# TaihuLight/Lol

Measured on AMD Instinct MI355X. Metric: cyclotomic poly-muls/sec (CRT·pointwise·CRT⁻¹), batched; bit-exact vs CT, higher is better.
Workload: dtype u64

## Files before the change

lol_amd/csrc/capi.cpp:

```cpp
#include <hip/hip_runtime_api.h>

#include <atomic>
#include <cstdlib>
#include <cstring>
#include <map>
#include <memory>
#include <mutex>
#include <string>
#include <vector>

#include "kernels.h"
#include "she_host.h"

using namespace lolhip;

namespace lolhip {
namespace {
const char* const kSwitchNames[SW_COUNT] = {"GENERIC_SCALAR", "NO_FUSED2", "NO_POW2_PART", "POLYMUL_UNFUSED",
                                            "KEYSWITCH_UNFUSED", "NO_T1", "NO_PIPE", "FORCE_PIPE", "NO_OWN_DIAG", "NO_MERGE", "NO_LAZY", "NO_KRON", "NO_TRUNC", "ELT_GLOBAL", "LPRF_VALU", "RLWE_RING_UNFUSED", "GAUSS_DENSE", "ZQ_DENSE_VALU", "ZQ_DENSE_MFMA", "CPLX_DENSE", "CPLX_DENSE_VALU", "ZQ_SCAN"};
std::atomic<int> g_switch[SW_COUNT];
std::once_flag g_switch_once;
void switches_init() {
  std::call_once(g_switch_once, [] {
    for (int i = 0; i < SW_COUNT; ++i) {
// ... 77 lines not shown
int zq_dense_route(const Plan& P, const StageProgram& sp) {
  if (!(P.routes & LOLHIP_ROUTE_DENSE_ZQ) || P.zq_mats.empty() || sw(SW_GENERIC_SCALAR)) return 0;
  if (use_mixed(P, sp) || sp.stages.size() > (size_t)ZQ_MAX_STAGES) return 0;
  int dmax = 0;
  for (const Stage& st : sp.stages) if (zq_dense_stage(st) && st.d > dmax) dmax = st.d;
  if (!dmax) return 0;
  return (P.zq_W && (dmax >= ZQ_MFMA_MIN_D || sw(SW_ZQ_DENSE_MFMA)) && !sw(SW_ZQ_DENSE_VALU)) ? 2 : 1;
}
const ZqDenseMat* zq_mat_of(const Plan& P, const Stage& st) {
  if (zq_dense_stage(st)) for (const ZqDenseMat& zm : P.zq_mats) if (zm.mat_off == st.mat_off) return &zm;
  return nullptr;
}

void zq_fill(const Plan& P, const StageProgram& sp, size_t at, ZqDenseLaunch& z) {
  z.W = P.zq_W; z.fold = P.zq_fold;
  z.mt = P.d_zq_mt; z.mtpc = P.zq_mt_per_comp;
  z.planes = P.d_zq_planes; z.plpc = P.zq_pl_per_comp;
  for (size_t i = 0; i < sp.stages.size(); ++i) {
    const Stage& st = sp.stages[i];
    const ZqDenseMat* zm = zq_mat_of(P, st);
    if (zm && st.d > z.dmax) z.dmax = st.d;
    z.kind[at + i] = !zm ? ZQ_ELT : st.rts >= 64 ? ZQ_COLS : ZQ_ROWS;
    z.mt_off[at + i] = zm ? zm->mt_off : -1; z.dp[at + i] = zm ? zm->dp : 0; z.pl_off[at + i] = zm ? zm->pl_off : -1;
  }
}

int zq_scan_route(const Plan& P, const StageProgram& sp) {
  if (!(P.routes & LOLHIP_ROUTE_SCAN_ZQ) || sw(SW_GENERIC_SCALAR) || P.n > 8192) return 0;
  const bool forced = sw(SW_ZQ_SCAN);
  if ((!forced && use_mixed(P, sp)) || sp.stages.size() > (size_t)ZQ_MAX_STAGES) return 0;
  bool hit = false;
  for (const Stage& st : sp.stages) {
    if (zq_scan_stage(st)) hit = hit || st.p > 13 || forced;
    else if (st.kind != ST_DIAG && st.kind != ST_SCALE) return 0;
  }
  return hit ? 1 : 0;
}

bool q_below(const Plan& P, int bits) {
  for (u64 q : P.qs) if (q >> bits) return false;
  return true;
}

bool use_fused2(const Plan& P) {
  return !sw(SW_NO_FUSED2) && P.fused2 && use_mixed(P, P.prog_crt_fused) && use_mixed(P, P.prog_crtinv_fused);
}

int run_pow2(const Plan& P, int mode, hipStream_t s, int64_t* y, const int64_t* a, const int64_t* b, int64_t B) {
  Pow2Launch l;
  l.stream = s; l.y = y; l.a = a; l.b = b; l.B = B; l.T = P.T; l.L = P.pow2.L;
  l.mod = P.d_mod;
  if (P.pow2.arith32) {
    l.arith = P.pow2.arith32; l.tw_fwd = P.pow2.d_tw_fwd32; l.tw_inv = P.pow2.d_tw_inv32; l.scale = P.pow2.d_scale32;
  } else {
    l.arith = 1;
    for (u64 q : P.qs) if (q >= (1ull << 61) || !(q & 1)) l.arith = 0;
    l.tw_fwd = P.pow2.d_tw_fwd; l.tw_inv = P.pow2.d_tw_inv; l.scale = P.pow2.d_scale;
    l.trunc = (l.arith == 1 && mode == 2 && !sw(SW_NO_TRUNC)) ? 1 : 0;
  }
  return hip_status(launch_pow2(l, mode));
}

}

namespace lolhip {

int need_device(const Plan& P) {
  if (!P.device) return LOLHIP_ERR_NO_DEVICE;
  int dev = -1;
  if (hipGetDevice(&dev) != hipSuccess) return LOLHIP_ERR_HIP;
  if (dev != P.device_id) return LOLHIP_ERR_DEVICE;
  return LOLHIP_OK;
}

int need_device(const lolhip_plan* p) { return p ? need_device(p->P) : LOLHIP_ERR_INVALID; }

int run_prog(const Plan& P, const StageProgram& sp, hipStream_t s, int64_t* y, int64_t B, const int64_t* src) {
  const int scan = zq_scan_route(P, sp);
  if (!scan && use_mixed(P, sp)) return hip_status(launch_mixed(mixed_launch(P, s, y, src ? src : y, B, sp)));
  GenericLaunch a;
  a.stream = s; a.y = y; a.B = B; a.T = P.T; a.n = P.n;
  a.stages = sp.d_stages; a.nstages = sp.nstages;
  a.consts = P.d_consts; a.cpc = P.consts_per_comp; a.mod = P.d_mod;
  StreamBuf ring(s);
  a.scratch = nullptr; a.scratch_bytes = 0;
  if (P.needs_scratch && B > 0) {
    const i64 groups = B * P.T < 512 ? B * P.T : 512;
    a.scratch_bytes = (size_t)groups * 2 * (size_t)P.n * sizeof(u64);
    if (!ring.alloc(a.scratch_bytes)) return LOLHIP_ERR_HIP;
    a.scratch = (u64*)ring.p;
  }
  a.q32 = true;
  for (u64 q : P.qs) if (q >= ((u64)1 << 32)) a.q32 = false;
  if (scan) {
    a.scan.route = scan;
    a.scan.src = (src && src != y) ? src : nullptr;
    a.scan.host_stages = sp.stages.data();
    for (size_t i = 0; i < sp.stages.size(); ++i)
      a.scan.kind[i] = !zq_scan_stage(sp.stages[i]) ? ZS_ELT : sp.stages[i].rts >= 64 ? ZS_COLS : ZS_LANES;
    return hip_status(launch_generic(a));
  }
  a.zq.route = zq_dense_route(P, sp);
  if (a.zq.route) {
    zq_fill(P, sp, 0, a.zq);
    a.zq.src = (src && src != y) ? src : nullptr;
    return hip_status(launch_generic(a));
// ... 919 lines not shown
```

lol_amd/csrc/plan.cpp:

```cpp
#include "plan.h"

#include <hip/hip_runtime_api.h>

#include <cmath>
#include <complex>
#include <cstring>

#include "kernels.h"
#include "lolhip.h"

namespace lolhip {

namespace {

template <typename E>
struct PoolBuilderT {
  int T;
  std::vector<std::vector<E>> pool;
  explicit PoolBuilderT(int T_) : T(T_), pool((size_t)T_) {}
  int size() const { return (int)pool[0].size(); }
  int add(const std::vector<std::vector<E>>& tab) {
    int off = size();
    for (int t = 0; t < T; ++t) pool[(size_t)t].insert(pool[(size_t)t].end(), tab[(size_t)t].begin(), tab[(size_t)t].end());
    return off;
// ... 743 lines not shown
    const Stage& st = P.prog_gauss.stages[si];
    if (st.wp_off) P.prog_gauss.nstages |= (st.rts >= 64 ? GAUSS_COLS : GAUSS_ROWS) << (8 + 2 * (int)si);
  }
  if ((rc = P.d_gcrt.upload(P.gcrt))) return rc;
  if ((rc = P.d_ginvcrt.upload(P.ginvcrt))) return rc;
  if ((rc = P.d_lift.upload(P.lift_consts))) return rc;

  if (P.is_pow2 || P.pow2_part) {
    const int L = P.pow2.L;
    const i64 n = (i64)1 << L;
    std::vector<u64> fwd((size_t)(T * n * 2), 0), inv((size_t)(T * n * 2), 0), sc((size_t)(T * 12), 0);
    for (int t = 0; t < T; ++t) {
      const u64 q = P.qs[(size_t)t];
      const u64 S = (u64)P.mhatinv[(size_t)t];
      {
        const u64 w1 = mulmod((u64)P.ruinv[0][(size_t)((n >> 1) * T + t)], S, q);
        const u64 R = (u64)((((unsigned __int128)1) << 64) % q);
        const u64 vals[4] = {S, w1, mulmod(S, R, q), mulmod(w1, R, q)};
        for (int k = 0; k < 4; ++k) {
          ShoupW ss = make_shoup(vals[k], q);
          sc[(size_t)(t * 8 + 2 * k)] = ss.w; sc[(size_t)(t * 8 + 2 * k + 1)] = ss.wp;
        }
        if (L >= 2) {
          const u64 S4 = mulmod(vals[2], 4 % q, q);
          const u64 tv[2] = {S4, mulmod(vals[3], 4 % q, q)};
          for (int k = 0; k < 2; ++k) {
            ShoupW ss = make_shoup(tv[k], q);
            sc[(size_t)(T * 8 + t * 4 + 2 * k)] = ss.w; sc[(size_t)(T * 8 + t * 4 + 2 * k + 1)] = ss.wp;
          }
        }
      }
      for (int s = 1; s <= L; ++s) {
        const i64 N = (i64)1 << s, half = N >> 1, step = n / N;
        for (i64 i = 0; i < half; ++i) {
          const i64 ex = step * (2 * i + 1);
          u64 w = (u64)P.ru[0][(size_t)(ex * T + t)];
          u64 wi = (u64)P.ruinv[0][(size_t)(ex * T + t)];
          if (s == 1) wi = mulmod(wi, S, q);
          ShoupW a = make_shoup(w, q), b = make_shoup(wi, q);
          const size_t o = ((size_t)t * n + (size_t)(half + i)) * 2;
          fwd[o] = a.w; fwd[o + 1] = a.wp;
          inv[o] = b.w; inv[o + 1] = b.wp;
        }
      }
    }
    if ((rc = P.pow2.d_tw_fwd.upload(fwd))) return rc;
    if ((rc = P.pow2.d_tw_inv.upload(inv))) return rc;
    if ((rc = P.pow2.d_scale.upload(sc))) return rc;
    P.pow2.arith32 = 4;
    for (u64 q : P.qs) { if (q >= (1ull << 27)) P.pow2.arith32 = 2; }
    for (u64 q : P.qs) { if (q >= (1ull << 30)) P.pow2.arith32 = 3; }
    for (u64 q : P.qs) { if (q >= (1ull << 31) || !(q & 1)) P.pow2.arith32 = 0; }
    if (P.pow2.arith32) {
      std::vector<uint32_t> f32(fwd.size()), i32(inv.size()), s32((size_t)T * 8);
      for (int t = 0; t < T; ++t) {
        const u64 q = P.qs[(size_t)t];
        for (i64 i = 0; i < n; ++i) {
          const size_t o = ((size_t)t * n + (size_t)i) * 2;
          f32[o] = (uint32_t)fwd[o]; f32[o + 1] = (uint32_t)((fwd[o] << 32) / q);
          i32[o] = (uint32_t)inv[o]; i32[o + 1] = (uint32_t)((inv[o] << 32) / q);
        }
        for (int k = 0; k < 4; ++k) {
          s32[(size_t)t * 8 + 2 * k] = (uint32_t)sc[(size_t)t * 8 + 2 * k];
          s32[(size_t)t * 8 + 2 * k + 1] = (uint32_t)((sc[(size_t)t * 8 + 2 * k] << 32) / q);
        }
      }
      if ((rc = P.pow2.d_tw_fwd32.upload(f32))) return rc;
      if ((rc = P.pow2.d_tw_inv32.upload(i32))) return rc;
      if ((rc = P.pow2.d_scale32.upload(s32))) return rc;
    }
  }
  P.needs_scratch = 2 * (size_t)P.n * sizeof(u64) > 152 * 1024;
  if (P.mixed_cls == 2 || P.mixed_cls == 4 || P.mixed_cls == 3) {
    const int sh = P.mixed_cls == 3 ? 64 : 32;
    std::vector<u64> mont(P.host_consts.size());
    for (int t = 0; t < T; ++t) {
      const u64 q = P.qs[(size_t)t];
      const u64 r = (u64)((((unsigned __int128)1) << sh) % q);
      for (int i = 0; i < P.consts_per_comp; ++i) {
        const size_t o = (size_t)t * P.consts_per_comp + i;
        mont[o] = mulmod(P.host_consts[o] % q, r, q);
      }
    }
    if ((rc = P.d_consts_mont.upload(mont))) return rc;
    if (P.mixed_cls == 2 || P.mixed_cls == 4) {
      std::vector<uint32_t> c32(mont.begin(), mont.end());
      if ((rc = P.d_consts32.upload(c32))) return rc;
    }
  }
  if (P.mixed_cls == 1) {
    std::vector<uint32_t> c32(P.host_consts.size());
    for (int t = 0; t < T; ++t)
      for (int i = 0; i < P.consts_per_comp; ++i) {
        const size_t o = (size_t)t * P.consts_per_comp + i;
        c32[o] = (uint32_t)(P.host_consts[o] % P.qs[(size_t)t]);
      }
    if ((rc = P.d_consts32.upload(c32))) return rc;
  }
  if (hipGetDevice(&P.device_id) != hipSuccess) return LOLHIP_ERR_HIP;
  P.device = true;
  return LOLHIP_OK;
}

}
```

lol_amd/csrc/pow2_impl.h:

```cpp
#pragma once
#include <hip/hip_runtime.h>

#include <atomic>
#include <mutex>
#include <type_traits>
#include <utility>

#include "kernels.h"
#include "zq_dev.h"

namespace lolhip {


constexpr int R = 4;
constexpr int E = 1 << R;
constexpr int LEVEL_PARTS = 4;

struct Lay {
  int reg[R];
  int thr[12];
  int ntb;
};
constexpr bool lay_eq(const Lay& a, const Lay& b) {
  if (a.ntb != b.ntb) return false;
// ... 489 lines not shown
    if (L < 10) return lay_std(L, L - R);
    int thr[12] = {0, 1, 2, 3, 4, 5, 10, 11, 12, 13, 14, 15};
    return lay_make(L, 6, 7, 8, 9, thr);
  }
  static constexpr Lay final_layout() { return HAS_G ? g() : wave_end(); }
};

template <int AR, bool INV, Lay A, int K0, int K1 = R>
__device__ __forceinline__ void fetch4(LevelTwT<VT<AR>> (&t)[R], const TwCtxT<VT<AR>>& tw, int xt) {
  if constexpr (K0 <= 0 && K1 > 0) tw_fetch<INV, A, 0>(t[0], tw, xt);
  if constexpr (K0 <= 1 && K1 > 1) tw_fetch<INV, A, 1>(t[1], tw, xt);
  if constexpr (K0 <= 2 && K1 > 2) tw_fetch<INV, A, 2>(t[2], tw, xt);
  if constexpr (K0 <= 3 && K1 > 3) tw_fetch<INV, A, 3>(t[3], tw, xt);
}
template <int AR, bool INV, Lay A, int K>
__device__ __forceinline__ void level_jit(VT<AR> (&v)[E], const TwCtxT<VT<AR>>& tw, int xt, const auto& qk) {
  using LevelTw = LevelTwT<VT<AR>>;
  if constexpr (tw_distinct(A, K) == 8 && sizeof(VT<AR>) == 8) {
    [&]<int... PART>(std::integer_sequence<int, PART...>) {
      (([&] { LevelTw t; tw_fetch<INV, A, K, PART>(t, tw, xt); level<AR, INV, A, K, PART>(v, t, tw, qk); }()), ...);
    }(std::make_integer_sequence<int, LEVEL_PARTS>{});
  } else {
    LevelTw t; tw_fetch<INV, A, K>(t, tw, xt); level<AR, INV, A, K>(v, t, tw, qk);
  }
}
template <int AR, Lay A, int K0, int K1 = R>
__device__ __forceinline__ void levels4_jit(VT<AR> (&v)[E], const TwCtxT<VT<AR>>& tw, int xt, const auto& qk) {
  if constexpr (K0 <= 0 && K1 > 0) level_jit<AR, false, A, 0>(v, tw, xt, qk);
  if constexpr (K0 <= 1 && K1 > 1) level_jit<AR, false, A, 1>(v, tw, xt, qk);
  if constexpr (K0 <= 2 && K1 > 2) level_jit<AR, false, A, 2>(v, tw, xt, qk);
  if constexpr (K0 <= 3 && K1 > 3) level_jit<AR, false, A, 3>(v, tw, xt, qk);
}
template <int AR, bool INV, Lay A, int K0, int K1 = R>
__device__ __forceinline__ void levels4(VT<AR> (&v)[E], const LevelTwT<VT<AR>> (&t)[R], const TwCtxT<VT<AR>>& tw, const auto& qk) {
  if constexpr (!INV) {
    if constexpr (K0 <= 0 && K1 > 0) level<AR, false, A, 0>(v, t[0], tw, qk);
    if constexpr (K0 <= 1 && K1 > 1) level<AR, false, A, 1>(v, t[1], tw, qk);
    if constexpr (K0 <= 2 && K1 > 2) level<AR, false, A, 2>(v, t[2], tw, qk);
    if constexpr (K0 <= 3 && K1 > 3) level<AR, false, A, 3>(v, t[3], tw, qk);
  } else {
    if constexpr (K0 <= 3 && K1 > 3) level<AR, true, A, 3>(v, t[3], tw, qk);
    if constexpr (K0 <= 2 && K1 > 2) level<AR, true, A, 2>(v, t[2], tw, qk);
    if constexpr (K0 <= 1 && K1 > 1) level<AR, true, A, 1>(v, t[1], tw, qk);
    if constexpr (K0 <= 0 && K1 > 0) level<AR, true, A, 0>(v, t[0], tw, qk);
  }
}

__device__ __forceinline__ int fresh(int x) {
  asm volatile("" : "+v"(x));
  return x;
}

struct NoTop {};
template <int AR, int L, Lay PREV, bool LEAN = false, bool W16 = false, typename TOP = NoTop, bool TRUNC = false>
__device__ __forceinline__ void fwd_transform(VT<AR> (&v)[E], VT<AR>* lds, const TwCtxT<VT<AR>>& tw, int tau_in, const auto& qk,
                                              TOP* pre = nullptr) {
  constexpr bool PRE = !std::is_same_v<TOP, NoTop>;
  using LevelTw = LevelTwT<VT<AR>>;
  using S = Sched<L, W16>;
  static_assert(!TRUNC || (L >= 11 && !PRE), "the truncated forward transform needs the G layout");
  constexpr int GK1 = TRUNC ? 2 : R;
  constexpr bool L10 = !(TRUNC && L == 11);
  {
    constexpr Lay A = S::w0();
    const int tau = fresh(tau_in);
    if constexpr (S::HAS_G && !lay_eq(PREV, A)) __syncthreads();
    transpose_put<PREV, A, false>(v, lds, tau);
    if constexpr (LEAN) {
      transpose_get<PREV, A, false>(v, lds, tau);
      levels4_jit<AR, A, 0>(v, tw, xthr<A>(tau), qk);
    } else {
      LevelTw t[R];
      fetch4<AR, false, A, 0>(t, tw, xthr<A>(tau));
      transpose_get<PREV, A, false>(v, lds, tau);
      levels4<AR, false, A, 0>(v, t, tw, qk);
    }
  }
  if constexpr (S::HAS_W1) {
    constexpr Lay A = S::w1();
    const int tau = fresh(tau_in);
    if constexpr (LEAN) {
      transpose_put<S::w0(), A, false>(v, lds, tau);
      transpose_get<S::w0(), A, false>(v, lds, tau);
      levels4_jit<AR, A, S::W1_K0>(v, tw, xthr<A>(tau), qk);
      if constexpr (S::NSWAP >= 1) { lane_swap<4, 3>(v); level_jit<AR, false, S::w1a(), 3>(v, tw, xthr<S::w1a()>(tau), qk); }
      if constexpr (S::NSWAP >= 2) {
        lane_swap<5, 2>(v);
        if constexpr (PRE) { pre->wait_l10(); level<AR, false, S::w1b(), 2>(v, pre->l10, tw, qk); }
        else if constexpr (L10) level_jit<AR, false, S::w1b(), 2>(v, tw, xthr<S::w1b()>(tau), qk);
      }
    } else {
      LevelTw t[R];
      transpose_put<S::w0(), A, false>(v, lds, tau);
      fetch4<AR, false, A, S::W1_K0>(t, tw, xthr<A>(tau));
      transpose_get<S::w0(), A, false>(v, lds, tau);
      if constexpr (S::W1_K0 <= 0) level<AR, false, A, 0>(v, t[0], tw, qk);
      if constexpr (S::W1_K0 <= 1) level<AR, false, A, 1>(v, t[1], tw, qk);
      if constexpr (S::W1_K0 <= 2) level<AR, false, A, 2>(v, t[2], tw, qk);
      LevelTw ua, ub;
      if constexpr (S::NSWAP >= 1) tw_fetch<false, S::w1a(), 3>(ua, tw, xthr<S::w1a()>(tau));
      level<AR, false, A, 3>(v, t[3], tw, qk);
      if constexpr (S::NSWAP >= 2 && !PRE && L10) tw_fetch<false, S::w1b(), 2>(ub, tw, xthr<S::w1b()>(tau));
      if constexpr (S::NSWAP >= 1) { lane_swap<4, 3>(v); level<AR, false, S::w1a(), 3>(v, ua, tw, qk); }
      if constexpr (S::NSWAP >= 2) {
        lane_swap<5, 2>(v);
        if constexpr (PRE) { pre->wait_l10(); level<AR, false, S::w1b(), 2>(v, pre->l10, tw, qk); }
        else if constexpr (L10) level<AR, false, S::w1b(), 2>(v, ub, tw, qk);
      }
    }
  }
  if constexpr (S::HAS_G) {
    constexpr Lay A = S::g();
    const int tau = fresh(tau_in);
    transpose_put<S::wave_end(), A, false>(v, lds, tau);
    if constexpr (PRE) {
      transpose_get<S::wave_end(), A, true>(v, lds, tau);
      pre->wait_g();
      levels4<AR, false, A, S::G_K0>(v, pre->g, tw, qk);
    } else if constexpr (LEAN) {
      transpose_get<S::wave_end(), A, true>(v, lds, tau);
      levels4_jit<AR, A, S::G_K0, GK1>(v, tw, xthr<A>(tau), qk);
    } else {
      LevelTw t[R];
      fetch4<AR, false, A, S::G_K0, GK1>(t, tw, xthr<A>(tau));
      transpose_get<S::wave_end(), A, true>(v, lds, tau);
      levels4<AR, false, A, S::G_K0, GK1>(v, t, tw, qk);
    }
  }
}

template <int AR, int L, Lay NEXT, bool W16 = false, bool TRUNC = false>
__device__ __forceinline__ void inv_transform(VT<AR> (&v)[E], VT<AR>* lds, const TwCtxT<VT<AR>>& tw, int tau_in, const auto& qk) {
  using LevelTw = LevelTwT<VT<AR>>;
  using S = Sched<L, W16>;
  static_assert(!TRUNC || L >= 11, "the truncated inverse transform needs the G layout");
  constexpr int GK1 = TRUNC ? 2 : R;
  constexpr bool L10 = !(TRUNC && L == 11);
  if constexpr (S::HAS_G) {
    constexpr Lay A = S::g();
    const int tau = fresh(tau_in);
    LevelTw t[R];
    fetch4<AR, true, A, S::G_K0, GK1>(t, tw, xthr<A>(tau));
    levels4<AR, true, A, S::G_K0, GK1>(v, t, tw, qk);
    transpose_put<A, S::wave_end(), true>(v, lds, tau);
  }
  if constexpr (S::HAS_W1) {
    constexpr Lay A = S::w1();
    const int tau = fresh(tau_in);
    const int xt = xthr<A>(tau);
    LevelTw ua, ub, t[R];
    if constexpr (S::NSWAP >= 2 && L10) tw_fetch<true, S::w1b(), 2>(ub, tw, xthr<S::w1b()>(tau));
    if constexpr (S::NSWAP >= 1) tw_fetch<true, S::w1a(), 3>(ua, tw, xthr<S::w1a()>(tau));
    if constexpr (S::NSWAP == 0) fetch4<AR, true, A, S::W1_K0>(t, tw, xt);
    if constexpr (S::HAS_G) transpose_get<S::g(), S::wave_end(), true>(v, lds, tau);
    if constexpr (S::NSWAP >= 2) { if constexpr (L10) level<AR, true, S::w1b(), 2>(v, ub, tw, qk); lane_swap<5, 2>(v); }
    if constexpr (S::NSWAP >= 1) {
      tw_fetch<true, A, 3>(t[3], tw, xt);
      level<AR, true, S::w1a(), 3>(v, ua, tw, qk);
      lane_swap<4, 3>(v);
      tw_fetch<true, A, 2>(t[2], tw, xt);
      tw_fetch<true, A, 1>(t[1], tw, xt);
      tw_fetch<true, A, 0>(t[0], tw, xt);
    }
    levels4<AR, true, A, S::W1_K0>(v, t, tw, qk);
    transpose_put<A, S::w0(), false>(v, lds, tau);
  }
  {
    constexpr Lay A = S::w0();
    const int tau = fresh(tau_in);
    LevelTw t[R];
    fetch4<AR, true, A, 0>(t, tw, xthr<A>(tau));
    if constexpr (S::HAS_W1) transpose_get<S::w1(), A, false>(v, lds, tau);
    levels4<AR, true, A, 0>(v, t, tw, qk);
    transpose_put<A, NEXT, false>(v, lds, tau);
    transpose_get<A, NEXT, false>(v, lds, tau);
  }
}


__device__ __forceinline__ void dot4_cols(const u64 (&x)[4], const u64 (&y)[4], u64& A, u64& B1, u64& B2, u64& C) {
  u64 k1, k2, k3, sj;
  u32 cnt;
  asm("v_mad_u64_u32 %[C], %[sj], %[x0l], %[y0l], 0\n\t"
      "v_mad_u64_u32 %[A], %[sj], %[x0h], %[y0h], 0\n\t"
      "v_mad_u64_u32 %[B1], %[sj], %[x0l], %[y0h], 0\n\t"
      "v_mad_u64_u32 %[C], %[k1], %[x1l], %[y1l], %[C]\n\t"
      "v_mad_u64_u32 %[B2], %[sj], %[x0h], %[y0l], 0\n\t"
      "v_mad_u64_u32 %[A], %[sj], %[x1h], %[y1h], %[A]\n\t"
      "v_cndmask_b32_e64 %[cnt], 0, 1, %[k1]\n\t"
      "v_mad_u64_u32 %[C], %[k2], %[x2l], %[y2l], %[C]\n\t"
// ... 1 lines not shown
      "v_mad_u64_u32 %[B2], %[sj], %[x1h], %[y1l], %[B2]\n\t"
      "v_addc_co_u32_e64 %[cnt], %[sj], %[cnt], 0, %[k2]\n\t"
      "v_mad_u64_u32 %[C], %[k3], %[x3l], %[y3l], %[C]\n\t"
      "v_mad_u64_u32 %[A], %[sj], %[x2h], %[y2h], %[A]\n\t"
      "v_mad_u64_u32 %[B1], %[sj], %[x2l], %[y2h], %[B1]\n\t"
      "v_addc_co_u32_e64 %[cnt], %[sj], %[cnt], 0, %[k3]\n\t"
      "v_mad_u64_u32 %[B2], %[sj], %[x2h], %[y2l], %[B2]\n\t"
      "v_mad_u64_u32 %[A], %[sj], %[x3h], %[y3h], %[A]\n\t"
      "v_mad_u64_u32 %[B1], %[sj], %[x3l], %[y3h], %[B1]\n\t"
      "v_mad_u64_u32 %[B2], %[sj], %[x3h], %[y3l], %[B2]\n\t"
      "v_mad_u64_u32 %[A], %[sj], %[cnt], 1, %[A]"
      : [A] "=&v"(A), [B1] "=&v"(B1), [B2] "=&v"(B2), [C] "=&v"(C), [cnt] "=&v"(cnt),
        [k1] "=&s"(k1), [k2] "=&s"(k2), [k3] "=&s"(k3), [sj] "=&s"(sj)
      : [x0l] "v"(lo32(x[0])), [x0h] "v"(hi32(x[0])), [x1l] "v"(lo32(x[1])), [x1h] "v"(hi32(x[1])),
        [x2l] "v"(lo32(x[2])), [x2h] "v"(hi32(x[2])), [x3l] "v"(lo32(x[3])), [x3h] "v"(hi32(x[3])),
        [y0l] "v"(lo32(y[0])), [y0h] "v"(hi32(y[0])), [y1l] "v"(lo32(y[1])), [y1h] "v"(hi32(y[1])),
        [y2l] "v"(lo32(y[2])), [y2h] "v"(hi32(y[2])), [y3l] "v"(lo32(y[3])), [y3h] "v"(hi32(y[3])));
}
__device__ __forceinline__ u64 dot4_redc(const u64 (&x)[4], const u64 (&y)[4], const ModCtx& mc) {
  u64 A, B1, B2, C;
  dot4_cols(x, y, A, B1, B2, C);
  const u64 u = (u64)hi32(C) + lo32(B1) + lo32(B2);
  const u64 lo = ((u64)lo32(u) << 32) | lo32(C);
  const u64 hi = A + hi32(B1) + hi32(B2) + hi32(u);
  return hi + __umul64hi(lo * mc.nqinv, mc.q) + (lo != 0);
}
template <Lay G>
__device__ __forceinline__ void pow2_base4(u64 (&v)[E], const u64 (&va)[E], const TwCtxT<u64>& tw, int xt, const ModCtx& mc, const QK& qk) {
  LevelTwT<u64> z;
  tw_fetch<false, G, 1>(z, tw, xt);
#pragma unroll
  for (int g = 0; g < 4; ++g) {
    constexpr int EK[4] = {0, 8, 4, 12};
    u64 zw = z.w[level_tab<G, 1>.slot[g & 1]], zwp = z.wp[level_tab<G, 1>.slot[g & 1]];
    if (g & 2) { zw = qk.q - zw; zwp = ~zwp; }
    u64 a[4], y[4];
#pragma unroll
    for (int k = 0; k < 4; ++k) {
      a[k] = va[g | EK[k]];
      y[k] = trim42(v[g | EK[k]], qk);
    }
#pragma unroll
    for (int k = 3; k >= 0; --k) {
      u64 x[4], w[4];
#pragma unroll
      for (int i = 0; i < 4; ++i) { x[i] = a[i]; w[i] = y[(k - i) & 3]; }
      v[g | EK[k]] = dot4_redc(x, w, mc);
      asm volatile("" : "+v"(v[g | EK[k]]));
      if (k) y[k] = trim2(shoup_acc<false>(y[k], zw, zwp, qk.nq, 0), qk);
    }
  }
}

constexpr int pow2_threads(int L) { return (1 << (L - R)) >= 256 ? (1 << (L - R)) : 256; }

template <int L, int MODE, int AR, bool T1 = false, bool TR = false>
__global__ void __launch_bounds__(pow2_threads(L), AR >= 2 ? 8 : 4)
k_pow2(i64* y, const i64* a_in, const i64* b_in, i64 B, int T,
       const VT<AR>* __restrict__ tw_fwd, const VT<AR>* __restrict__ tw_inv, const VT<AR>* __restrict__ scale,
       const ModCtx* __restrict__ mod, int xcd_map) {
  using S = Sched<L, T1>;
  using V = VT<AR>;
  static_assert(!TR || (MODE == 2 && AR == 1 && L >= 11), "the truncated route is the 61-bit fused poly-mul's");
  constexpr int n = 1 << L;
  constexpr int NT = 1 << (L - R);
  constexpr int PPW = NT >= 256 ? 1 : 256 / NT;
  constexpr int LDSW = n + n / 16 + twl_words(n);
  constexpr u32 TWB = 2 * sizeof(V);
  extern __shared__ __attribute__((aligned(16))) unsigned char smem[];
  V* lds = reinterpret_cast<V*>(smem) + (threadIdx.x / NT) * LDSW;
  V* lds_tw = lds + n + n / 16;
  const int tau = threadIdx.x % NT;
  if constexpr (T1) T = 1;

  const i64 item0 = (i64)blockIdx.x * PPW;
  const int slot = (PPW == 1) ? 0 : (int)(threadIdx.x / NT);
  const i64 item = item0 + slot;
  i64 b, b0; int t;
  if (xcd_map) { i64 g = item / (8 * (i64)T); int r = (int)(item % (8 * T)); b = g * 8 + (r & 7); t = r >> 3; b0 = b; }
  else { b = item / T; t = (int)(item % T); b0 = item0 / T; }
  if constexpr (T1) { b = item; t = 0; b0 = item0; }

  if constexpr (NT >= 64) {
    t = __builtin_amdgcn_readfirstlane(t);
    b = (i64)(((u64)(u32)__builtin_amdgcn_readfirstlane((int)(b >> 32)) << 32) | (u32)__builtin_amdgcn_readfirstlane((int)b));
  }
  b0 = (i64)(((u64)(u32)__builtin_amdgcn_readfirstlane((int)(b0 >> 32)) << 32) | (u32)__builtin_amdgcn_readfirstlane((int)b0));
  constexpr bool TIGHT = (AR == 1 && MODE == 2 && !(NT >= 64 || T1) && L >= 5);
  const QKT<AR, (NT >= 64 || T1), !TIGHT> qk(mod[t], std::bool_constant<(NT >= 64 || T1)>{});
  const u64 win = (u64)(B - b0) * n * T * 8;
  const u32 wbytes = win > 0xFFFFFFFFull ? 0xFFFFFFFFu : (u32)win;
  const size_t wbase = (size_t)b0 * n * T;
  const rsrc_t ry = __builtin_amdgcn_make_buffer_rsrc((void*)(y + wbase), 0, wbytes, 0x00020000);
  const rsrc_t ra = __builtin_amdgcn_make_buffer_rsrc((void*)(a_in + (MODE == 2 ? wbase : 0)), 0, MODE == 2 ? wbytes : 0, 0x00020000);
  const rsrc_t rb = __builtin_amdgcn_make_buffer_rsrc((void*)(b_in + (MODE == 2 ? wbase : 0)), 0, MODE == 2 ? wbytes : 0, 0x00020000);
  TwCtxT<V> tw;
  tw.fwd = __builtin_amdgcn_make_buffer_rsrc((void*)tw_fwd, 0, (u32)T * n * TWB, 0x00020000);
  tw.inv = __builtin_amdgcn_make_buffer_rsrc((void*)tw_inv, 0, (u32)T * n * TWB, 0x00020000);
  tw.comp = (u32)t * (u32)n * TWB;
  tw.pf = tw_fwd + (size_t)t * n * 2;
  if constexpr (!TIGHT) tw.pi = tw_inv + (size_t)t * n * 2;
  tw.lds_tw = lds_tw;
  if constexpr (L >= TWL_MIN_L) tw_fill_lds<NT>(lds_tw, (MODE == 1) ? tw.inv : tw.fwd, tw.comp, n, tau);
  constexpr int SC = (MODE == 2 && AR == 1) ? 4 : 0;
  const V* scp = TR ? scale + (size_t)T * 8 + (size_t)t * 4 : scale + (size_t)t * 8 + SC;
  if constexpr (!TIGHT) {
    tw.sc0 = scp[0];
    tw.sc1 = scp[1];
    tw.l1w = scp[2];
    tw.l1wp = scp[3];
  }

  constexpr Lay LIO = S::io();
  constexpr Lay LFIN = S::final_layout();
  const u32 uT8 = (u32)T * 8u;
  const u32 pofs = ((u32)(b - b0) * (u32)n * (u32)T + (u32)t) * 8u;
  const u32 off_io = pofs + (u32)xthr<LIO>(tau) * uT8;
  const u32 off_fin = pofs + (u32)xthr<LFIN>(tau) * uT8;

  V v[E];
  if constexpr (MODE == 0 || MODE == 2) {
    const rsrc_t src = (MODE == 2) ? ra : ry;
    load_poly<LIO, T1>(src, off_io, uT8, [&](int e, u64 x) { v[e] = from_i64_fwd<AR>((i64)x, qk); });
    fwd_transform<AR, L, LIO, TIGHT, T1, NoTop, TR>(v, lds, tw, tau, qk);
  }
  if constexpr (MODE == 2) {
    V va[E];
#pragma unroll
    for (int e = 0; e < E; ++e) {
      va[e] = park_fwd<AR>(v[e], qk);
      if constexpr (TR) asm volatile("" : "+v"(va[e]));
    }
    const bool square = (a_in == b_in);
    if (!square) {
      u64 raw[E];
      load_poly<LIO, T1>(rb, off_io, uT8, [&](int e, u64 x) { raw[e] = x; });
      __builtin_amdgcn_sched_barrier(0);
#pragma unroll
      for (int e = 0; e < E; ++e) v[e] = from_i64_fwd<AR>((i64)raw[e], qk);
      fwd_transform<AR, L, LIO, true, T1, NoTop, TR>(v, lds, tw, tau, qk);
    }
    const int tl = TIGHT ? fresh(t) : t;
    const ModCtx mc = mod[tl];
    if constexpr (TR) {
      pow2_base4<LFIN>(v, va, tw, xthr<LFIN>(fresh(tau)), mc, qk);
    } else {
#pragma unroll
      for (int e = 0; e < E; ++e) v[e] = pmul<AR>(va[e], (AR < 2 && square) ? va[e] : v[e], mc, qk);
    }
  }
  if constexpr (MODE == 2 && L >= TWL_MIN_L) {
    if constexpr (L > 10) __syncthreads();
    tw_fill_lds<NT>(lds_tw, tw.inv, tw.comp, n, tau);
  }
  if constexpr (MODE == 1) {
    load_poly<LFIN, T1>(ry, off_fin, uT8, [&](int e, u64 x) { v[e] = from_i64_inv<AR>((i64)x, qk); });
  }
  if constexpr (MODE == 0) {
    store_poly<LFIN, T1>(ry, off_fin, uT8, [&](int e) { return (u64)canon_fwd<AR>(v[e], qk); });
  } else {
    if constexpr (TIGHT) {
      const int tl = fresh(t);
      tw.pi = tw_inv + (size_t)tl * n * 2;
      const V* sc = scale + (size_t)tl * 8 + SC;
      tw.sc0 = sc[0];
      tw.sc1 = sc[1];
      tw.l1w = sc[2];
      tw.l1wp = sc[3];
    }
    inv_transform<AR, L, LIO, T1, TR>(v, lds, tw, tau, qk);
    store_poly<LIO, T1>(ry, off_io, uT8, [&](int e) { return (u64)canon_inv<AR>(v[e], qk); });
  }
}

constexpr int MAX_DEV = 64;
struct KernelDev { std::atomic<int> state{0}; };
inline std::mutex& kernel_dev_mutex() { static std::mutex m; return m; }
template <typename Setup>
static hipError_t kernel_dev_setup(KernelDev (&tab)[MAX_DEV], Setup&& setup) {
  int dev = -1;
  hipError_t e = hipGetDevice(&dev);
  if (e != hipSuccess) return e;
  if (dev < 0 || dev >= MAX_DEV) return hipErrorInvalidDevice;
  KernelDev& d = tab[dev];
  if (d.state.load(std::memory_order_acquire) != 2) {
    std::lock_guard<std::mutex> g(kernel_dev_mutex());
    if (d.state.load(std::memory_order_relaxed) != 2) {
      e = setup();
      if (e != hipSuccess) return e;
      d.state.store(2, std::memory_order_release);
    }
  }
  return hipSuccess;
}

template <int L, int MODE, int AR, bool T1, bool TR = false>
static hipError_t launch_pow2_L(const Pow2Launch& a) {
  if constexpr (MODE == 2 && AR == 1 && L >= 11 && !TR) {
    if (a.trunc) return launch_pow2_L<L, MODE, AR, T1, true>(a);
  }
  constexpr int n = 1 << L;
  constexpr int NT = 1 << (L - R);
  constexpr int PPW = NT >= 256 ? 1 : 256 / NT;
  constexpr int LDSW = n + n / 16 + twl_words(n);
  const size_t lds_bytes = (size_t)PPW * LDSW * sizeof(VT<AR>);
  const i64 items = a.B * a.T;
  const int xcd_map = (a.T > 1 && PPW == 1 && a.B % 8 == 0) ? 1 : 0;
  const i64 grid = (items + PPW - 1) / PPW;
  if (grid == 0) return hipSuccess;
  if (lds_bytes > 64 * 1024) {
    static KernelDev tab[MAX_DEV];
    hipError_t e = kernel_dev_setup(tab, [&]() -> hipError_t {
      return hipFuncSetAttribute(reinterpret_cast<const void*>(&k_pow2<L, MODE, AR, T1, TR>),
                                 hipFuncAttributeMaxDynamicSharedMemorySize, (int)lds_bytes);
    });
    if (e != hipSuccess) return e;
  }
  hipLaunchKernelGGL((k_pow2<L, MODE, AR, T1, TR>), dim3((unsigned)grid), dim3(NT * PPW), lds_bytes, a.stream,
                     a.y, a.a, a.b, a.B, a.T, static_cast<const VT<AR>*>(a.tw_fwd), static_cast<const VT<AR>*>(a.tw_inv),
                     static_cast<const VT<AR>*>(a.scale), a.mod, xcd_map);
  return hipGetLastError();
}

// ... 30 lines not shown
```

lol_amd/csrc/pow2_pipe.hip:

```cpp
#include "pow2_impl.h"
#include <cstdio>
#include <cstdlib>

namespace lolhip {

typedef __attribute__((address_space(3))) void lds_void_t;

__device__ __forceinline__ void dma_dword_asm(rsrc_t r, u32 lds_byte, u32 voff, u32 soff) {
  u32 keep;
  asm volatile("s_nop 4\n\ts_mov_b32 %0, m0\n\ts_mov_b32 m0, %1\n\ts_nop 0\n\tbuffer_load_dword %2, %3, %4 offen lds\n\ts_mov_b32 m0, %0"
               : "=&s"(keep) : "s"(lds_byte), "v"(voff), "s"(r), "s"(soff));
}
__device__ __forceinline__ u32x2 load_b64_asm(rsrc_t r, u32 voff, u32 soff) {
  u32x2 x;
  asm volatile("s_nop 4\n\tbuffer_load_dwordx2 %0, %1, %2, %3 offen" : "=v"(x) : "v"(voff), "s"(r), "s"(soff));
  return x;
}
template <Lay A, int K> struct TwRaw { u32x2 r[tw_distinct(A, K)]; };
template <Lay A, int K>
__device__ __forceinline__ void tw_issue(TwRaw<A, K>& raw, rsrc_t tab, int xt) {
  constexpr int beta = A.reg[K];
  const u32 voff = (u32)(xt & ((1 << beta) - 1)) * 8u;
  int ord = 0, j = 0;
#pragma unroll
  for (int e = 0; e < E; ++e) {
    if (e & (1 << K)) continue;
    if (level_tab<A, K>.slot[e] == ord) raw.r[j++] = load_b64_asm(tab, voff, (u32)level_tab<A, K>.cidx[e] * 8u);
    ++ord;
  }
}
template <Lay A, int K>
__device__ __forceinline__ void tw_landed(LevelTwT<u32>& t, TwRaw<A, K>& raw) {
#pragma unroll
  for (int j = 0; j < tw_distinct(A, K); ++j) asm volatile("" : "+v"(raw.r[j]));
  int ord = 0, j = 0;
#pragma unroll
  for (int e = 0; e < E; ++e) {
    if (e & (1 << K)) continue;
    if (level_tab<A, K>.slot[e] == ord) { t.w[ord] = raw.r[j].x; t.wp[ord] = raw.r[j].y; ++j; }
    ++ord;
  }
}
template <int L, int NDMA> struct PipeTop {
  using S = Sched<L, true>;
  static constexpr Lay AL = S::w1b(), AG = S::g();
  static constexpr int NG = (S::G_K0 <= 1 ? tw_distinct(AG, 1) : 0) + (S::G_K0 <= 2 ? tw_distinct(AG, 2) : 0) + tw_distinct(AG, 3);
  TwRaw<AL, 2> r10;
  TwRaw<AG, 1> rg1;
  TwRaw<AG, 2> rg2;
  TwRaw<AG, 3> rg3;
  LevelTwT<u32> l10, g[R];
  __device__ __forceinline__ void issue(rsrc_t tab, int tau) {
    static_assert(S::NSWAP == 2 && S::HAS_G && S::G_K0 >= 1, "n = 4096 or 8192");
    tw_issue(r10, tab, xthr<AL>(tau));
    const int xg = xthr<AG>(tau);
    if constexpr (S::G_K0 <= 1) tw_issue(rg1, tab, xg);
    if constexpr (S::G_K0 <= 2) tw_issue(rg2, tab, xg);
    tw_issue(rg3, tab, xg);
  }
  __device__ __forceinline__ void wait_l10() {
    asm volatile("s_waitcnt vmcnt(%0)" :: "n"(NG + NDMA));
    tw_landed(l10, r10);
  }
  __device__ __forceinline__ void wait_g() {
    asm volatile("s_waitcnt vmcnt(%0)" :: "n"(NDMA));
    if constexpr (S::G_K0 <= 1) tw_landed(g[1], rg1);
    if constexpr (S::G_K0 <= 2) tw_landed(g[2], rg2);
    tw_landed(g[3], rg3);
  }
};

constexpr int PIPE_ROW = 68;
constexpr int pipe_lds_words(int n) { return (n + n / 16) + 2 * twl_words(n) + (n / 64) * PIPE_ROW; }

template <int L, int AR, bool SQ>
__global__ void __launch_bounds__(1 << (L - R), 4)
k_pow2_pipe(i64* __restrict__ c, const i64* a, const i64* b, i64 B, const u32* __restrict__ tw_fwd, const u32* __restrict__ tw_inv,
            const u32* __restrict__ scale, const ModCtx* __restrict__ mod) {
  static_assert(AR >= 2 && L >= 12, "32-bit classes; one polynomial per workgroup of whole waves");
  using S = Sched<L, true>;
  using V = u32;
  constexpr int n = 1 << L;
  constexpr int NT = 1 << (L - R);
  constexpr int WORK = n + n / 16, TWW = twl_words(n);
  extern __shared__ __attribute__((aligned(16))) unsigned char smem[];
  V* lds = reinterpret_cast<V*>(smem);
  V* lds_twf = lds + WORK;
  V* lds_twi = lds_twf + TWW;
  V* stage = lds_twi + TWW;
  const int tau = threadIdx.x;
  const int lane = tau & 63;
  const int wv = __builtin_amdgcn_readfirstlane(tau >> 6);

  QK32 qk(mod[0], std::true_type{});
  asm volatile("" : "+v"(qk.q2));
  TwCtxT<V> twf;
  twf.fwd = __builtin_amdgcn_make_buffer_rsrc((void*)tw_fwd, 0, (u32)n * 8u, 0x00020000);
  twf.inv = __builtin_amdgcn_make_buffer_rsrc((void*)tw_inv, 0, (u32)n * 8u, 0x00020000);
  twf.comp = 0;
  twf.pf = tw_fwd;
  twf.pi = tw_inv;
  twf.lds_tw = lds_twf;
  twf.sc0 = scale[0]; twf.sc1 = scale[1]; twf.l1w = scale[2]; twf.l1wp = scale[3];
  TwCtxT<V> twi = twf;
  twi.lds_tw = lds_twi;
  tw_fill_lds<NT>(lds_twf, twf.fwd, 0, n, tau);
  tw_fill_lds<NT>(lds_twi, twf.inv, 0, n, tau);

  const u32* tw_fwd_opaque = tw_fwd;
  asm volatile("" : "+s"(tw_fwd_opaque));
  const rsrc_t tab_asm = __builtin_amdgcn_make_buffer_rsrc((void*)tw_fwd_opaque, 0, (u32)n * 8u, 0x00020000);
  V* wst = stage + wv * (16 * PIPE_ROW);
  const V* rd = wst + (lane >> 2) * PIPE_ROW + (lane & 3) * 16;
  const u32 wst_byte = __builtin_amdgcn_readfirstlane((u32)(size_t)wst);
  auto dma = [&](const i64* src, i64 poly) {
    const rsrc_t r = __builtin_amdgcn_make_buffer_rsrc((void*)(src + poly * n), 0, (u32)n * 8u, 0x00020000);
#pragma unroll
    for (int ch = 0; ch < 16; ++ch)
      dma_dword_asm(r, wst_byte + (u32)(ch * PIPE_ROW * 4), (u32)lane * 8u, (u32)(wv * 8192 + ch * 512));
  };
  const u32 rd_byte = (u32)(size_t)rd;
  auto take = [&](V (&v)[E]) {
    u32x4 w0, w1, w2, w3;
    asm volatile("s_waitcnt vmcnt(0)\n\tds_read_b128 %0, %4\n\tds_read_b128 %1, %4 offset:16\n\tds_read_b128 %2, %4 offset:32\n\t"
                 "ds_read_b128 %3, %4 offset:48\n\ts_waitcnt lgkmcnt(0)"
                 : "=&v"(w0), "=&v"(w1), "=&v"(w2), "=&v"(w3) : "v"(rd_byte));
    const u32x4 w[4] = {w0, w1, w2, w3};
#pragma unroll
    for (int k = 0; k < 4; ++k) { v[4 * k + 0] = w[k].x; v[4 * k + 1] = w[k].y; v[4 * k + 2] = w[k].z; v[4 * k + 3] = w[k].w; }
#pragma unroll
    for (int e = 0; e < E; ++e) v[e] = v[e] + qk.q;
  };

  constexpr Lay LIO = S::io();
  const u32 off_io = (u32)xthr<LIO>(tau) * 8u;
  const i64 G = gridDim.x;
  i64 p = blockIdx.x;
  if (p < B) dma(a, p);
  __syncthreads();
  for (; p < B; p += G) {
    V v[E], va[E];
    take(v);
    PipeTop<L, 16> top;
    top.issue(tab_asm, tau);
    const i64 pn = (p + G < B) ? p + G : p;
    if constexpr (SQ) dma(a, pn); else dma(b, p);
    fwd_transform<AR, L, S::w0(), false, true, PipeTop<L, 16>>(v, lds, twf, tau, qk, &top);
#pragma unroll
    for (int e = 0; e < E; ++e) va[e] = park_fwd<AR>(v[e], qk);
    if constexpr (!SQ) {
      __syncthreads();
      take(v);
      dma(a, pn);
      fwd_transform<AR, L, S::w0(), true, true, PipeTop<L, 16>>(v, lds, twf, tau, qk, &top);
    }
    const ModCtx mc = mod[0];
#pragma unroll
    for (int e = 0; e < E; ++e) v[e] = pmul<AR>(va[e], v[e], mc, qk);
    inv_transform<AR, L, LIO, true>(v, lds, twi, tau, qk);
    const rsrc_t rc = __builtin_amdgcn_make_buffer_rsrc((void*)(c + p * n), 0, (u32)n * 8u, 0x00020000);
    store_poly<LIO, true>(rc, off_io, 8u, [&](int e) { return (u64)canon_inv<AR>(v[e], qk); });
  }
  asm volatile("s_waitcnt vmcnt(0)");
}

template <int L, int AR, bool SQ>
static hipError_t launch_pipe_L(const Pow2Launch& a) {
  constexpr int n = 1 << L;
  constexpr int NT = 1 << (L - R);
  const size_t lds_bytes = (size_t)pipe_lds_words(n) * sizeof(u32);
  static KernelDev tab[MAX_DEV];
  static int cus[MAX_DEV];
  hipError_t e = kernel_dev_setup(tab, [&]() -> hipError_t {
    int dev = 0;
    hipError_t r = hipGetDevice(&dev);
    if (r != hipSuccess) return r;
    r = hipDeviceGetAttribute(&cus[dev], hipDeviceAttributeMultiprocessorCount, dev);
    if (r != hipSuccess) return r;
    return hipFuncSetAttribute(reinterpret_cast<const void*>(&k_pow2_pipe<L, AR, SQ>), hipFuncAttributeMaxDynamicSharedMemorySize, (int)lds_bytes);
  });
  if (e != hipSuccess) return e;
  int dev = 0;
  if ((e = hipGetDevice(&dev)) != hipSuccess) return e;
  int per_cu = 2 * (int)((80 * 1024) / lds_bytes);
  if (per_cu < 1) per_cu = 1;
  if (per_cu > 16 * 64 / NT) per_cu = 16 * 64 / NT;
  i64 grid = (i64)cus[dev] * per_cu;
  if (const char* g = getenv("LOLHIP_PIPE_GRID")) grid = atol(g);
  if (getenv("LOLHIP_PIPE_INFO")) {
    int occ = -1;
    hipError_t oe = hipOccupancyMaxActiveBlocksPerMultiprocessor(&occ, reinterpret_cast<const void*>(&k_pow2_pipe<L, AR, SQ>), NT, lds_bytes);
    fprintf(stderr, "k_pow2_pipe<%d,%d>: lds %zu B, per_cu %d, occupancy query %d (err %d), grid %lld\n", L, AR, lds_bytes, per_cu, occ, (int)oe, (long long)grid);
  }
  if (grid > a.B) grid = a.B;
  if (grid == 0) return hipSuccess;
  hipLaunchKernelGGL((k_pow2_pipe<L, AR, SQ>), dim3((unsigned)grid), dim3(NT), lds_bytes, a.stream, a.y, a.a, a.b, a.B,
                     static_cast<const u32*>(a.tw_fwd), static_cast<const u32*>(a.tw_inv), static_cast<const u32*>(a.scale), a.mod);
  return hipGetLastError();
}

bool pow2_pipe_ok(const Pow2Launch& a, bool forced) {
  if (a.T != 1 || a.arith < 2 || (a.L != 13 && !(forced && a.L == 12))) return false;
  if (((uintptr_t)a.y & 15) || (((uintptr_t)a.a | (uintptr_t)a.b) & 7)) return false;
  return forced || a.B >= 2048;
}

template <bool SQ> static hipError_t launch_pipe_sq(const Pow2Launch& a) {
  switch (a.arith * 100 + a.L) {
    case 212: return launch_pipe_L<12, 2, SQ>(a);
    case 213: return launch_pipe_L<13, 2, SQ>(a);
    case 312: return launch_pipe_L<12, 3, SQ>(a);
    case 313: return launch_pipe_L<13, 3, SQ>(a);
    case 412: return launch_pipe_L<12, 4, SQ>(a);
    case 413: return launch_pipe_L<13, 4, SQ>(a);
    default: return hipErrorInvalidValue;
  }
}
hipError_t launch_pow2_pipe(const Pow2Launch& a) { return a.a == a.b ? launch_pipe_sq<true>(a) : launch_pipe_sq<false>(a); }

}
```

Before: 9.973 million.

## Truncate NTT two levels and multiply degree-3 residues in 32-bit pipe kernel

Generalises the truncated-transform template parameter from a bool to a level count. The pipelined 32-bit power-of-two kernel now stops the forward NTT two levels early and replaces the pointwise product with a small schoolbook multiply of degree-3 residues mod x^4 - zeta, using a fused Montgomery reduction. Scale constants are adjusted on the host to match. This removes two butterfly levels each way and their twiddle loads, at the cost of more multiplies in the base case and new kernel instantiations.

Result: no change. 9.991 million, median of 2 (+0.2%).

```diff
diff --git a/lol_amd/csrc/capi.cpp b/lol_amd/csrc/capi.cpp
--- a/lol_amd/csrc/capi.cpp
+++ b/lol_amd/csrc/capi.cpp
@@ -153,6 +153,7 @@
   l.mod = P.d_mod;
   if (P.pow2.arith32) {
     l.arith = P.pow2.arith32; l.tw_fwd = P.pow2.d_tw_fwd32; l.tw_inv = P.pow2.d_tw_inv32; l.scale = P.pow2.d_scale32;
+    l.trunc = (mode == 2 && !sw(SW_NO_TRUNC)) ? 1 : 0;
   } else {
     l.arith = 1;
     for (u64 q : P.qs) if (q >= (1ull << 61) || !(q & 1)) l.arith = 0;
diff --git a/lol_amd/csrc/plan.cpp b/lol_amd/csrc/plan.cpp
--- a/lol_amd/csrc/plan.cpp
+++ b/lol_amd/csrc/plan.cpp
@@ -819,7 +819,7 @@
     for (u64 q : P.qs) { if (q >= (1ull << 30)) P.pow2.arith32 = 3; }
     for (u64 q : P.qs) { if (q >= (1ull << 31) || !(q & 1)) P.pow2.arith32 = 0; }
     if (P.pow2.arith32) {
-      std::vector<uint32_t> f32(fwd.size()), i32(inv.size()), s32((size_t)T * 8);
+      std::vector<uint32_t> f32(fwd.size()), i32(inv.size()), s32((size_t)T * 12, 0);
       for (int t = 0; t < T; ++t) {
         const u64 q = P.qs[(size_t)t];
         for (i64 i = 0; i < n; ++i) {
@@ -830,6 +830,13 @@
         for (int k = 0; k < 4; ++k) {
           s32[(size_t)t * 8 + 2 * k] = (uint32_t)sc[(size_t)t * 8 + 2 * k];
           s32[(size_t)t * 8 + 2 * k + 1] = (uint32_t)((sc[(size_t)t * 8 + 2 * k] << 32) / q);
+        }
+        if (L >= 2) {
+          const u64 tv[2] = {mulmod(sc[(size_t)t * 8], 4 % q, q), mulmod(sc[(size_t)t * 8 + 2], 4 % q, q)};
+          for (int k = 0; k < 2; ++k) {
+            s32[(size_t)T * 8 + (size_t)t * 4 + 2 * k] = (uint32_t)tv[k];
+            s32[(size_t)T * 8 + (size_t)t * 4 + 2 * k + 1] = (uint32_t)((tv[k] << 32) / q);
+          }
         }
       }
       if ((rc = P.pow2.d_tw_fwd32.upload(f32))) return rc;
diff --git a/lol_amd/csrc/pow2_impl.h b/lol_amd/csrc/pow2_impl.h
--- a/lol_amd/csrc/pow2_impl.h
+++ b/lol_amd/csrc/pow2_impl.h
@@ -565,15 +565,15 @@
 }
 
 struct NoTop {};
-template <int AR, int L, Lay PREV, bool LEAN = false, bool W16 = false, typename TOP = NoTop, bool TRUNC = false>
+template <int AR, int L, Lay PREV, bool LEAN = false, bool W16 = false, typename TOP = NoTop, int TRUNC = 0>
 __device__ __forceinline__ void fwd_transform(VT<AR> (&v)[E], VT<AR>* lds, const TwCtxT<VT<AR>>& tw, int tau_in, const auto& qk,
                                               TOP* pre = nullptr) {
   constexpr bool PRE = !std::is_same_v<TOP, NoTop>;
   using LevelTw = LevelTwT<VT<AR>>;
   using S = Sched<L, W16>;
-  static_assert(!TRUNC || (L >= 11 && !PRE), "the truncated forward transform needs the G layout");
-  constexpr int GK1 = TRUNC ? 2 : R;
-  constexpr bool L10 = !(TRUNC && L == 11);
+  static_assert(TRUNC == 0 || (L >= 11 && TRUNC <= 3 && L - TRUNC >= 9), "the truncated forward transform needs the G layout");
+  constexpr int GK1 = R - TRUNC;
+  constexpr bool L10 = L - TRUNC >= 10;
   {
     constexpr Lay A = S::w0();
     const int tau = fresh(tau_in);
@@ -599,7 +599,7 @@
       if constexpr (S::NSWAP >= 1) { lane_swap<4, 3>(v); level_jit<AR, false, S::w1a(), 3>(v, tw, xthr<S::w1a()>(tau), qk); }
       if constexpr (S::NSWAP >= 2) {
         lane_swap<5, 2>(v);
-        if constexpr (PRE) { pre->wait_l10(); level<AR, false, S::w1b(), 2>(v, pre->l10, tw, qk); }
+        if constexpr (PRE && L10) { pre->wait_l10(); level<AR, false, S::w1b(), 2>(v, pre->l10, tw, qk); }
         else if constexpr (L10) level_jit<AR, false, S::w1b(), 2>(v, tw, xthr<S::w1b()>(tau), qk);
       }
     } else {
@@ -617,7 +617,7 @@
       if constexpr (S::NSWAP >= 1) { lane_swap<4, 3>(v); level<AR, false, S::w1a(), 3>(v, ua, tw, qk); }
       if constexpr (S::NSWAP >= 2) {
         lane_swap<5, 2>(v);
-        if constexpr (PRE) { pre->wait_l10(); level<AR, false, S::w1b(), 2>(v, pre->l10, tw, qk); }
+        if constexpr (PRE && L10) { pre->wait_l10(); level<AR, false, S::w1b(), 2>(v, pre->l10, tw, qk); }
         else if constexpr (L10) level<AR, false, S::w1b(), 2>(v, ub, tw, qk);
       }
     }
@@ -629,7 +629,7 @@
     if constexpr (PRE) {
       transpose_get<S::wave_end(), A, true>(v, lds, tau);
       pre->wait_g();
-      levels4<AR, false, A, S::G_K0>(v, pre->g, tw, qk);
+      levels4<AR, false, A, S::G_K0, GK1>(v, pre->g, tw, qk);
     } else if constexpr (LEAN) {
       transpose_get<S::wave_end(), A, true>(v, lds, tau);
       levels4_jit<AR, A, S::G_K0, GK1>(v, tw, xthr<A>(tau), qk);
@@ -642,13 +642,13 @@
   }
 }
 
-template <int AR, int L, Lay NEXT, bool W16 = false, bool TRUNC = false>
+template <int AR, int L, Lay NEXT, bool W16 = false, int TRUNC = 0>
 __device__ __forceinline__ void inv_transform(VT<AR> (&v)[E], VT<AR>* lds, const TwCtxT<VT<AR>>& tw, int tau_in, const auto& qk) {
   using LevelTw = LevelTwT<VT<AR>>;
   using S = Sched<L, W16>;
-  static_assert(!TRUNC || L >= 11, "the truncated inverse transform needs the G layout");
-  constexpr int GK1 = TRUNC ? 2 : R;
-  constexpr bool L10 = !(TRUNC && L == 11);
+  static_assert(TRUNC == 0 || (L >= 11 && TRUNC <= 3 && L - TRUNC >= 9), "the truncated inverse transform needs the G layout");
+  constexpr int GK1 = R - TRUNC;
+  constexpr bool L10 = L - TRUNC >= 10;
   if constexpr (S::HAS_G) {
     constexpr Lay A = S::g();
     const int tau = fresh(tau_in);
@@ -756,6 +756,47 @@
   }
 }
 
+__device__ __forceinline__ u32 redc32(u64 x, const QK32& k) {
+  const u32 m = (u32)x * k.nqinv;
+  return (u32)((x + (u64)m * k.q) >> 32);
+}
+template <Lay G, int AR, int D>
+__device__ __forceinline__ void pow2_base32(u32 (&v)[E], const u32 (&va)[E], const LevelTwT<u32>& z, const QK32& qk) {
+  static_assert(AR >= 2 && D == 2 && G.reg[2] == G.reg[1] + 1 && G.reg[3] == G.reg[1] + 2, "degree-3 residues on register bits 2, 3 of G");
+#pragma unroll
+  for (int g = 0; g < 4; ++g) {
+    constexpr int EK[4] = {0, 8, 4, 12};
+    u32 zw = z.w[level_tab<G, 1>.slot[g & 1]], zwp = z.wp[level_tab<G, 1>.slot[g & 1]];
+    if (g & 2) { zw = qk.q - zw; zwp = ~zwp; }
+    u32 a[4], y[4];
+#pragma unroll
+    for (int k = 0; k < 4; ++k) {
+      a[k] = va[g | EK[k]];
+      const u32 b = v[g | EK[k]];
+      y[k] = AR == 4 ? b : AR == 2 ? csub32(b, qk.q2) : csub32(b, qk.q);
+    }
+#pragma unroll
+    for (int k = 3; k >= 0; --k) {
+      u32 w[4];
+#pragma unroll
+      for (int i = 0; i < 4; ++i) w[i] = y[(k - i) & 3];
+      u32 t;
+      if constexpr (AR == 3) {
+        const u32 t0 = csub32(redc32((u64)a[0] * w[0] + (u64)a[1] * w[1], qk), qk.q);
+        const u32 t1 = csub32(redc32((u64)a[2] * w[2] + (u64)a[3] * w[3], qk), qk.q);
+        t = csub32(t0 + t1, qk.q);
+      } else {
+        t = csub32(redc32((u64)a[0] * w[0] + (u64)a[1] * w[1] + (u64)a[2] * w[2] + (u64)a[3] * w[3], qk), qk.q2);
+      }
+      v[g | EK[k]] = t;
+      if (k) {
+        const u32 zb = shoup32(y[k], zw, zwp, qk.q);
+        y[k] = AR == 3 ? csub32(zb, qk.q) : zb;
+      }
+    }
+  }
+}
+
 constexpr int pow2_threads(int L) { return (1 << (L - R)) >= 256 ? (1 << (L - R)) : 256; }
 
 template <int L, int MODE, int AR, bool T1 = false, bool TR = false>
@@ -826,7 +867,7 @@
   if constexpr (MODE == 0 || MODE == 2) {
     const rsrc_t src = (MODE == 2) ? ra : ry;
     load_poly<LIO, T1>(src, off_io, uT8, [&](int e, u64 x) { v[e] = from_i64_fwd<AR>((i64)x, qk); });
-    fwd_transform<AR, L, LIO, TIGHT, T1, NoTop, TR>(v, lds, tw, tau, qk);
+    fwd_transform<AR, L, LIO, TIGHT, T1, NoTop, TR ? 2 : 0>(v, lds, tw, tau, qk);
   }
   if constexpr (MODE == 2) {
     V va[E];
@@ -842,7 +883,7 @@
       __builtin_amdgcn_sched_barrier(0);
 #pragma unroll
       for (int e = 0; e < E; ++e) v[e] = from_i64_fwd<AR>((i64)raw[e], qk);
-      fwd_transform<AR, L, LIO, true, T1, NoTop, TR>(v, lds, tw, tau, qk);
+      fwd_transform<AR, L, LIO, true, T1, NoTop, TR ? 2 : 0>(v, lds, tw, tau, qk);
     }
     const int tl = TIGHT ? fresh(t) : t;
     const ModCtx mc = mod[tl];
@@ -872,7 +913,7 @@
       tw.l1w = sc[2];
       tw.l1wp = sc[3];
     }
-    inv_transform<AR, L, LIO, T1, TR>(v, lds, tw, tau, qk);
+    inv_transform<AR, L, LIO, T1, TR ? 2 : 0>(v, lds, tw, tau, qk);
     store_poly<LIO, T1>(ry, off_io, uT8, [&](int e) { return (u64)canon_inv<AR>(v[e], qk); });
   }
 }
diff --git a/lol_amd/csrc/pow2_pipe.hip b/lol_amd/csrc/pow2_pipe.hip
--- a/lol_amd/csrc/pow2_pipe.hip
+++ b/lol_amd/csrc/pow2_pipe.hip
@@ -70,16 +70,40 @@
   }
 };
 
+template <int L, int NDMA> struct PipeTopTr {
+  using S = Sched<L, true>;
+  static constexpr Lay AL = S::w1b(), AG = S::g();
+  static constexpr int NG = tw_distinct(AG, 1);
+  TwRaw<AL, 2> r10;
+  TwRaw<AG, 1> rg1;
+  LevelTwT<u32> l10, g[R];
+  __device__ __forceinline__ void issue(rsrc_t tab, int tau) {
+    static_assert(S::NSWAP == 2 && S::HAS_G && S::G_K0 >= 1 && L - 2 >= 10, "n = 4096 or 8192");
+    tw_issue(r10, tab, xthr<AL>(tau));
+    tw_issue(rg1, tab, xthr<AG>(tau));
+  }
+  __device__ __forceinline__ void wait_l10() {
+    asm volatile("s_waitcnt vmcnt(%0)" :: "n"(NG + NDMA));
+    tw_landed(l10, r10);
+  }
+  __device__ __forceinline__ void wait_g() {
+    asm volatile("s_waitcnt vmcnt(%0)" :: "n"(NDMA));
+    tw_landed(g[1], rg1);
+  }
+};
+
 constexpr int PIPE_ROW = 68;
 constexpr int pipe_lds_words(int n) { return (n + n / 16) + 2 * twl_words(n) + (n / 64) * PIPE_ROW; }
 
-template <int L, int AR, bool SQ>
+template <int L, int AR, bool SQ, bool TR = false>
 __global__ void __launch_bounds__(1 << (L - R), 4)
 k_pow2_pipe(i64* __restrict__ c, const i64* a, const i64* b, i64 B, const u32* __restrict__ tw_fwd, const u32* __restrict__ tw_inv,
             const u32* __restrict__ scale, const ModCtx* __restrict__ mod) {
   static_assert(AR >= 2 && L >= 12, "32-bit classes; one polynomial per workgroup of whole waves");
   using S = Sched<L, true>;
   using V = u32;
+  using Top = std::conditional_t<TR, PipeTopTr<L, 16>, PipeTop<L, 16>>;
+  constexpr int TD = TR ? 2 : 0;
   constexpr int n = 1 << L;
   constexpr int NT = 1 << (L - R);
   constexpr int WORK = n + n / 16, TWW = twl_words(n);
@@ -101,7 +125,8 @@
   twf.pf = tw_fwd;
   twf.pi = tw_inv;
   twf.lds_tw = lds_twf;
-  twf.sc0 = scale[0]; twf.sc1 = scale[1]; twf.l1w = scale[2]; twf.l1wp = scale[3];
+  const u32* scp = scale + (TR ? 8 : 0);
+  twf.sc0 = scp[0]; twf.sc1 = scp[1]; twf.l1w = scp[2]; twf.l1wp = scp[3];
   TwCtxT<V> twi = twf;
   twi.lds_tw = lds_twi;
   tw_fill_lds<NT>(lds_twf, twf.fwd, 0, n, tau);
@@ -141,31 +166,38 @@
   for (; p < B; p += G) {
     V v[E], va[E];
     take(v);
-    PipeTop<L, 16> top;
+    Top top;
     top.issue(tab_asm, tau);
     const i64 pn = (p + G < B) ? p + G : p;
     if constexpr (SQ) dma(a, pn); else dma(b, p);
-    fwd_transform<AR, L, S::w0(), false, true, PipeTop<L, 16>>(v, lds, twf, tau, qk, &top);
+    fwd_transform<AR, L, S::w0(), false, true, Top, TD>(v, lds, twf, tau, qk, &top);
 #pragma unroll
     for (int e = 0; e < E; ++e) va[e] = park_fwd<AR>(v[e], qk);
     if constexpr (!SQ) {
       __syncthreads();
       take(v);
       dma(a, pn);
-      fwd_transform<AR, L, S::w0(), true, true, PipeTop<L, 16>>(v, lds, twf, tau, qk, &top);
+      fwd_transform<AR, L, S::w0(), true, true, Top, TD>(v, lds, twf, tau, qk, &top);
     }
-    const ModCtx mc = mod[0];
-#pragma unroll
-    for (int e = 0; e < E; ++e) v[e] = pmul<AR>(va[e], v[e], mc, qk);
-    inv_transform<AR, L, LIO, true>(v, lds, twi, tau, qk);
+    if constexpr (TR) {
+      pow2_base32<S::g(), AR, TD>(v, va, top.g[1], qk);
+    } else {
+      const ModCtx mc = mod[0];
+#pragma unroll
+      for (int e = 0; e < E; ++e) v[e] = pmul<AR>(va[e], v[e], mc, qk);
+    }
+    inv_transform<AR, L, LIO, true, TD>(v, lds, twi, tau, qk);
     const rsrc_t rc = __builtin_amdgcn_make_buffer_rsrc((void*)(c + p * n), 0, (u32)n * 8u, 0x00020000);
     store_poly<LIO, true>(rc, off_io, 8u, [&](int e) { return (u64)canon_inv<AR>(v[e], qk); });
   }
   asm volatile("s_waitcnt vmcnt(0)");
 }
 
-template <int L, int AR, bool SQ>
+template <int L, int AR, bool SQ, bool TR = false>
 static hipError_t launch_pipe_L(const Pow2Launch& a) {
+  if constexpr (!TR) {
+    if (a.trunc) return launch_pipe_L<L, AR, SQ, true>(a);
+  }
   constexpr int n = 1 << L;
   constexpr int NT = 1 << (L - R);
   const size_t lds_bytes = (size_t)pipe_lds_words(n) * sizeof(u32);
@@ -177,7 +209,7 @@
     if (r != hipSuccess) return r;
     r = hipDeviceGetAttribute(&cus[dev], hipDeviceAttributeMultiprocessorCount, dev);
     if (r != hipSuccess) return r;
-    return hipFuncSetAttribute(reinterpret_cast<const void*>(&k_pow2_pipe<L, AR, SQ>), hipFuncAttributeMaxDynamicSharedMemorySize, (int)lds_bytes);
+    return hipFuncSetAttribute(reinterpret_cast<const void*>(&k_pow2_pipe<L, AR, SQ, TR>), hipFuncAttributeMaxDynamicSharedMemorySize, (int)lds_bytes);
   });
   if (e != hipSuccess) return e;
   int dev = 0;
@@ -189,12 +221,12 @@
   if (const char* g = getenv("LOLHIP_PIPE_GRID")) grid = atol(g);
   if (getenv("LOLHIP_PIPE_INFO")) {
     int occ = -1;
-    hipError_t oe = hipOccupancyMaxActiveBlocksPerMultiprocessor(&occ, reinterpret_cast<const void*>(&k_pow2_pipe<L, AR, SQ>), NT, lds_bytes);
-    fprintf(stderr, "k_pow2_pipe<%d,%d>: lds %zu B, per_cu %d, occupancy query %d (err %d), grid %lld\n", L, AR, lds_bytes, per_cu, occ, (int)oe, (long long)grid);
+    hipError_t oe = hipOccupancyMaxActiveBlocksPerMultiprocessor(&occ, reinterpret_cast<const void*>(&k_pow2_pipe<L, AR, SQ, TR>), NT, lds_bytes);
+    fprintf(stderr, "k_pow2_pipe<%d,%d>: lds %zu B, per_cu %d, occupancy query %d (err %d), grid %lld, trunc %d\n", L, AR, lds_bytes, per_cu, occ, (int)oe, (long long)grid, TR ? 2 : 0);
   }
   if (grid > a.B) grid = a.B;
   if (grid == 0) return hipSuccess;
-  hipLaunchKernelGGL((k_pow2_pipe<L, AR, SQ>), dim3((unsigned)grid), dim3(NT), lds_bytes, a.stream, a.y, a.a, a.b, a.B,
+  hipLaunchKernelGGL((k_pow2_pipe<L, AR, SQ, TR>), dim3((unsigned)grid), dim3(NT), lds_bytes, a.stream, a.y, a.a, a.b, a.B,
                      static_cast<const u32*>(a.tw_fwd), static_cast<const u32*>(a.tw_inv), static_cast<const u32*>(a.scale), a.mod);
   return hipGetLastError();
 }
```
